# EugenHotaj/pytorch-generative

Measured on AMD Instinct MI355X. Metric: training images/sec (ImageGPT 8-block/4-head/16-embed, 28x28x1), higher is better.
Workload: dtype f32; 1 GPU; BASELINE.json configs[1]: ImageGPT 8 blocks / 4 heads / 16 embed on 28x28x1 binarised-MNIST-shaped synthetic; one step = zero_grad + fwd + BCE + bwd + global grad-norm + Adam + lr decay (reference trainer.py:173-193); per_gpu_batch=1024, global_batch=1024, parallelism=dp1, launch=hipGraph replay

## Files before the change

### include/pg_hip.h

```cpp
#ifndef PG_HIP_H_
#define PG_HIP_H_

#include <stddef.h>
#include <stdint.h>

#ifdef __cplusplus
extern "C" {
#endif

#define PG_ABI_VERSION 2

#define PG_EINVAL (-1)
#define PG_ESHAPE (-2)

#define PG_MAX_TAPS 64

#define PG_ACT_NONE 0
#define PG_ACT_RELU 1
#define PG_ACT_ELU 2
#define PG_ACT_GELU 3
#define PG_ACT_ELU_OUT 4

#define PG_GATE_TANH 0
#define PG_GATE_IDENTITY 1
// ... 170 lines not shown
                    void* stream);
size_t pg_mlp_gelu_bwd_workspace_floats(int N, int L);

int pg_gpt_block_head_fwd(const float* x, const float* ln_w, const float* ln_b, const float* wq,
                          const float* bq, const float* wkv, const float* bkv, float* qkv, int N,
                          int C, int L, float eps, void* stream);
int pg_gpt_block_head_bwd(const float* x, const float* ln_w, const float* ln_b, const float* wq,
                          const float* wkv, const float* dqkv, const float* gx, float* dx,
                          float* dln_w, float* dln_b, float* dwq, float* dbq, float* dwkv,
                          float* dbkv, int N, int C, int L, float eps, float* workspace,
                          size_t workspace_floats, void* stream);
size_t pg_gpt_block_head_bwd_workspace_floats(int N, int L);
int pg_gpt_block_tail_fwd(const float* o, const float* x, const float* wp, const float* bp,
                          const float* ln_w, const float* ln_b, const float* w1, const float* b1,
                          const float* w2, const float* b2, float* x_new, int N, int C, int Hd,
                          int L, float eps, void* stream);
int pg_gpt_block_tail_bwd(const float* o, const float* x, const float* wp, const float* bp,
                          const float* ln_w, const float* ln_b, const float* w1, const float* b1,
                          const float* w2, const float* dx_new, float* d_o, float* gx, float* dwp,
                          float* dbp, float* dln_w, float* dln_b, float* dw1, float* db1,
                          float* dw2, float* db2, int N, int C, int Hd, int L, float eps,
                          float* workspace, size_t workspace_floats, void* stream);
size_t pg_gpt_block_tail_bwd_workspace_floats(int N, int L);
int pg_gpt_block_tail_bwd_partial(const float* o, const float* x, const float* wp, const float* bp,
                                  const float* ln_w, const float* ln_b, const float* w1, const float* b1,
                                  const float* w2, const float* dx_new, float* d_o, float* gx, int N, int Cc,
                                  int Hd, int L, float eps, float* workspace, size_t workspace_floats,
                                  void* stream);
int pg_gpt_block_head_bwd_with_tail(const float* x, const float* ln_w, const float* ln_b, const float* wq,
                                    const float* wkv, const float* dqkv, const float* gx, float* dx,
                                    float* dln_w, float* dln_b, float* dwq, float* dbq, float* dwkv,
                                    float* dbkv, int N, int Cc, int L, float eps, float* workspace,
                                    size_t workspace_floats, const float* tail_workspace, float* t_dw1,
                                    float* t_db1, float* t_dw2, float* t_db2, float* t_dwp, float* t_dbp,
                                    float* t_dln_w, float* t_dln_b, void* stream);
int pg_gpt_block_head_bwd_partial(const float* x, const float* ln_w, const float* ln_b, const float* wq, const float* wkv,
                                  const float* dqkv, const float* gx, float* dx, int N, int C, int L, float eps,
                                  float* workspace, size_t workspace_floats, void* stream);
int pg_gpt_blocks_reduce(int n_blocks, const float* const* head_ws, const float* const* tail_ws, float* const* grads,
                         int N, int C, int L, void* stream);

int pg_sample_embed(const float* canvas, const float* pos, const float* w, const float* b, float* out,
                    int N, int Cin, int H, int W, int Cout, int KH, int KW, int r, int c, int ld,
                    const int* pos_dev, void* stream);
int pg_attn_decode(const float* qkv, float* k_cache, float* v_cache, float* o, int N, int heads,
                   int L, int p, int dk, int dv, int ld, int strict, const int* pos_dev,
// ... 76 lines not shown
```

### pytorch-generative_amd/csrc/gpt_block.hip

```cpp
#include <stdlib.h>

#include "common.h"
#include "gpt_ends.h"

namespace {

typedef float f32x4 __attribute__((ext_vector_type(4)));
#define MFMA16(A, B, C) __builtin_amdgcn_mfma_f32_16x16x4f32((A), (B), (C), 0, 0, 0)

constexpr int C = 16, HD = 64, QKV = 48;
constexpr int GB_THREADS = 256;
constexpr int TS = 20;
constexpr float INV_C = 1.f / 16.f;

constexpr int TB_WAVE_ROWS = 2 * HD + 4 * C;
constexpr int T_W1 = 0, T_B1 = T_W1 + HD * C, T_W2 = T_B1 + HD, T_B2 = T_W2 + C * HD, T_WP = T_B2 + C,
              T_BP = T_WP + C * C, T_G2 = T_BP + C, T_BE2 = T_G2 + C, T_PART = T_BE2 + C;
constexpr int H_WQ = 0, H_WKV = H_WQ + C * C, H_BQ = H_WKV + 2 * C * C, H_BKV = H_BQ + C,
              H_G1 = H_BKV + 2 * C, H_BE1 = H_G1 + C, H_PART = H_BE1 + C;

struct BlockArgs {
  const float* x; const float* g1; const float* be1; const float* wq; const float* bq;
  const float* wkv; const float* bkv; float* qkv; const float* dqkv; const float* gx; float* dx;
  const float* o; const float* wp; const float* bp; const float* g2; const float* be2;
// ... 59 lines not shown
};
__device__ __forceinline__ void prefetch_fence() { __builtin_amdgcn_sched_barrier(0); }
constexpr int waitcnt_gfx9(int vm, int exp, int lgkm) { return ((vm & 0x30) << 10) | (vm & 0xF) | ((exp & 7) << 4) | ((lgkm & 0xF) << 8); }
#if defined(__HIP_DEVICE_COMPILE__) && !defined(__GFX9__)
#error "wait_prologue_loads() encodes s_waitcnt for gfx9; re-derive the immediate for another target"
#endif
__device__ __forceinline__ void wait_prologue_loads() {
  constexpr int VMCNT0_ONLY = waitcnt_gfx9( 0,  7,  15);
  static_assert(VMCNT0_ONLY == 0x0F70, "gfx9 s_waitcnt vmcnt(0)");
  __builtin_amdgcn_s_waitcnt(VMCNT0_ONLY);
}
__device__ __forceinline__ void lds_put_tile(float* t, int j, int g, const f32x4& v) {
#pragma unroll
  for (int r = 0; r < 4; ++r) t[(4 * g + r) * TS + j] = v[r];
}
__device__ __forceinline__ f32x4 lds_row4(const float* t, int row, int g) {
  return *reinterpret_cast<const f32x4*>(t + row * TS + 4 * g);
}

__device__ __forceinline__ const float* qkv_row(const BlockArgs& a, int ch) {
  return ch < C ? a.wq + ch * C : a.wkv + (ch - C) * C;
}

__global__ void __launch_bounds__(GB_THREADS) head_fwd_kernel(const BlockArgs a) {
  const int lane = threadIdx.x & 63, j = lane & 15, g = lane >> 4;
  const int wave = blockIdx.x * (GB_THREADS / 64) + __builtin_amdgcn_readfirstlane(threadIdx.x >> 6);
  const int nwaves = gridDim.x * (GB_THREADS / 64);
  float wf[3][4];
  f32x4 bias[3];
#pragma unroll
  for (int m = 0; m < 3; ++m) {
#pragma unroll
    for (int r = 0; r < 4; ++r) {
      wf[m][r] = qkv_row(a, 16 * m + j)[4 * g + r];
      const int ch = 16 * m + 4 * g + r;
      bias[m][r] = ch < C ? a.bq[ch] : a.bkv[ch - C];
    }
  }
  const f32x4 gam = load_vec(a.g1, g), bet = load_vec(a.be1, g);
  if (wave >= a.total_tiles) return;
  TileWalk tw(a, wave, nwaves);
  f32x4 xv = load_tile(a.x + tw.base(C, a.L) + j, a.L, g);
  wait_prologue_loads();
  for (;;) {
    const TileWalk nx = tw.next();
    const bool more = nx.n < a.N;
    const f32x4 xn = load_tile(a.x + (more ? nx : tw).base(C, a.L) + j, a.L, g);
    prefetch_fence();
    const Ln s = ln_stats(xv, a.eps);
    f32x4 y;
#pragma unroll
    for (int r = 0; r < 4; ++r) y[r] = fmaf(s.xhat[r], gam[r], bet[r]);
    float* qb = a.qkv + tw.base(QKV, a.L) + j;
#pragma unroll
    for (int m = 0; m < 3; ++m) {
      f32x4 out = bias[m];
#pragma unroll
      for (int r = 0; r < 4; ++r) out = MFMA16(wf[m][r], y[r], out);
      store_tile(qb + (size_t)(16 * m) * a.L, a.L, g, out);
    }
    if (!more) break;
    xv = xn;
    tw = nx;
  }
}

__global__ void __launch_bounds__(GB_THREADS) head_bwd_kernel(const BlockArgs a) {
  extern __shared__ float4 lds4[];
  float* lds = reinterpret_cast<float*>(lds4);
  const int lane = threadIdx.x & 63, j = lane & 15, g = lane >> 4;
  const int wv = __builtin_amdgcn_readfirstlane(threadIdx.x >> 6);
  const int wave = blockIdx.x * (GB_THREADS / 64) + wv;
  const int nwaves = gridDim.x * (GB_THREADS / 64);
  float* ty = lds + (size_t)wv * (C + QKV) * TS;
  float* tq = ty + C * TS;

  float wt[3][4];
#pragma unroll
  for (int m = 0; m < 3; ++m) {
#pragma unroll
    for (int r = 0; r < 4; ++r) wt[m][r] = qkv_row(a, 16 * m + 4 * g + r)[j];
  }
  const f32x4 gam = load_vec(a.g1, g), bet = load_vec(a.be1, g);
// ... 67 lines not shown
  __syncthreads();
  float* mine = lds + (size_t)wv * H_PART;
#pragma unroll
  for (int m = 0; m < 3; ++m) {
#pragma unroll
    for (int r = 0; r < 4; ++r) {
      const int ch = 16 * m + 4 * g + r;
      mine[H_WQ + ch * C + j] = accw[m][r];
      const float b = jsum16(accb[m][r]);
      if (j == 0) mine[H_BQ + ch] = b;
    }
  }
#pragma unroll
  for (int r = 0; r < 4; ++r) {
    const float dg = jsum16(dgam[r]), db = jsum16(dbet[r]);
    if (j == 0) { mine[H_G1 + 4 * g + r] = dg; mine[H_BE1 + 4 * g + r] = db; }
  }
  __syncthreads();
  float* prow = a.part + (size_t)blockIdx.x * H_PART;
  for (int i = threadIdx.x; i < H_PART; i += GB_THREADS)
    prow[i] = (lds[i] + lds[H_PART + i]) + (lds[2 * H_PART + i] + lds[3 * H_PART + i]);
}

__global__ void __launch_bounds__(GB_THREADS) tail_fwd_kernel(const BlockArgs a) {
  const int lane = threadIdx.x & 63, j = lane & 15, g = lane >> 4;
  const int wave = blockIdx.x * (GB_THREADS / 64) + __builtin_amdgcn_readfirstlane(threadIdx.x >> 6);
  const int nwaves = gridDim.x * (GB_THREADS / 64);
  float wpf[4], w1f[4][4], w2f[4][4];
  f32x4 b1r[4];
#pragma unroll
  for (int r = 0; r < 4; ++r) wpf[r] = a.wp[j * C + 4 * g + r];
#pragma unroll
  for (int m = 0; m < 4; ++m) {
#pragma unroll
    for (int r = 0; r < 4; ++r) {
      w1f[m][r] = a.w1[(16 * m + j) * C + 4 * g + r];
      w2f[m][r] = a.w2[j * HD + 16 * m + 4 * g + r];
      b1r[m][r] = a.b1[16 * m + 4 * g + r];
    }
  }
  const f32x4 bpv = load_vec(a.bp, g), b2v = load_vec(a.b2, g);
  const f32x4 gam = load_vec(a.g2, g), bet = load_vec(a.be2, g);
  if (wave >= a.total_tiles) return;
  TileWalk tw(a, wave, nwaves);
  size_t off = tw.base(C, a.L) + j;
  f32x4 xv = load_tile(a.x + off, a.L, g);
  f32x4 ov = load_tile(a.o + off, a.L, g);
  wait_prologue_loads();
  for (;;) {
    const TileWalk nx = tw.next();
    const bool more = nx.n < a.N;
    const size_t offn = (more ? nx : tw).base(C, a.L) + j;
    const f32x4 xn = load_tile(a.x + offn, a.L, g);
    const f32x4 on = load_tile(a.o + offn, a.L, g);
    prefetch_fence();
    f32x4 xm = xv + bpv;
#pragma unroll
    for (int r = 0; r < 4; ++r) xm = MFMA16(wpf[r], ov[r], xm);
    const Ln s = ln_stats(xm, a.eps);
    f32x4 y;
#pragma unroll
    for (int r = 0; r < 4; ++r) y[r] = fmaf(s.xhat[r], gam[r], bet[r]);
    f32x4 h[4];
#pragma unroll
    for (int m = 0; m < 4; ++m) {
      h[m] = b1r[m];
#pragma unroll
      for (int r = 0; r < 4; ++r) h[m] = MFMA16(w1f[m][r], y[r], h[m]);
    }
    f32x4 out = (xm + b2v) + xv;
#pragma unroll
    for (int m = 0; m < 4; ++m) {
#pragma unroll
      for (int r = 0; r < 4; ++r) out = MFMA16(w2f[m][r], gelu_f(h[m][r]), out);
    }
    store_tile(a.xnew + off, a.L, g, out);
    if (!more) break;
    xv = xn;
    ov = on;
    off = offn;
    tw = nx;
  }
}

__global__ void __launch_bounds__(GB_THREADS) tail_bwd_kernel(const BlockArgs a) {
  extern __shared__ float4 lds4[];
  float* lds = reinterpret_cast<float*>(lds4);
  const int lane = threadIdx.x & 63, j = lane & 15, g = lane >> 4;
  const int wv = __builtin_amdgcn_readfirstlane(threadIdx.x >> 6);
  const int wave = blockIdx.x * (GB_THREADS / 64) + wv;
  const int nwaves = gridDim.x * (GB_THREADS / 64);
  float* tg = lds + (size_t)wv * TB_WAVE_ROWS * TS;
  float* th = tg + HD * TS;
  float* ty = th + HD * TS;
  float* tx = ty + C * TS;
  float* td = tx + C * TS;
  float* to = td + C * TS;

  float* wl = lds + (size_t)4 * TB_WAVE_ROWS * TS;
// ... 289 lines not shown
      const float* p = a.part + col[k];
      int r = rg;
      for (; r + 32 < a.rows; r += 64) {
        a0 += p[(size_t)r * a.stride];
        a1 += p[(size_t)(r + 32) * a.stride];
      }
      if (r < a.rows) a0 += p[(size_t)r * a.stride];
    }
  }
  red[rg][sl] = a0 + a1;
  __syncthreads();
  if (rg != 0 || s >= ncol) return;
  float acc = 0.f;
#pragma unroll
  for (int r = 0; r < 32; ++r) acc += red[r][sl];
  int begin = 0;
  for (int k = 0; k < a.nseg; ++k) {
    if (s < a.end[k]) { a.dst[k][s - begin] += acc; return; }
    begin = a.end[k];
  }
}

int grid_blocks(int which, int N, int L) {
  struct Cfg { int cap[4]; int mt[2]; };
  static const Cfg cfg = []() {
    Cfg c = {{2048, 1024, 2048, 512},
             {1, 2}};
    if (const char* e = PG_AB_ENV("PG_BLOCK_GRID")) {
      int v[4];
      if (sscanf(e, "%d,%d,%d,%d", &v[0], &v[1], &v[2], &v[3]) == 4 && v[0] > 0 && v[1] > 0 && v[2] > 0 && v[3] > 0)
        for (int i = 0; i < 4; ++i) c.cap[i] = v[i];
    }
    if (const char* e = PG_AB_ENV("PG_BLOCK_MINTILES")) {
      int f = 0, b = 0;
      if (sscanf(e, "%d,%d", &f, &b) == 2 && f > 0 && b > 0) { c.mt[0] = f; c.mt[1] = b; }
    }
    return c;
  }();
  const int* cap = cfg.cap;
  const int* mt_cfg = cfg.mt;
  const int min_tiles = (which & 1) ? mt_cfg[1] : mt_cfg[0];
  const long tiles = (long)N * (L / 16);
  long b = (tiles + 4 * min_tiles - 1) / (4 * min_tiles);
  if (b > cap[which]) b = cap[which];
  return b < 1 ? 1 : (int)b;
}
int bwd_blocks(int N, int L) { return grid_blocks(3, N, L); }

int check_shape(const char* who, int N, int Cc, int L) {
  PG_REQUIRE(N > 0 && L > 0, PG_EINVAL, "%s: non-positive dimension", who);
  PG_REQUIRE(Cc == C, PG_ESHAPE, "%s: only C = 16 is instantiated (got %d)", who, Cc);
  PG_REQUIRE(L % 16 == 0, PG_ESHAPE, "%s: L=%d is not a multiple of 16", who, L);
  return 0;
}
// ... 198 lines not shown
  }
  an.n = nj;
  an.first[nj] = nb;
  hipLaunchKernelGGL(seg_reduceM_kernel, dim3((unsigned)nb), dim3(256), 0, (hipStream_t)stream, an);
  PG_LAUNCH_CHECK("pg_gpt_model_reduce");
  return 0;
}

PG_EXPORT int pg_gpt_block_tail_fwd(const float* o, const float* x, const float* wp, const float* bp,
                                    const float* ln_w, const float* ln_b, const float* w1, const float* b1,
                                    const float* w2, const float* b2, float* x_new, int N, int Cc, int Hd,
                                    int L, float eps, void* stream) {
  PG_REQUIRE(o && x && wp && bp && ln_w && ln_b && w1 && b1 && w2 && b2 && x_new, PG_EINVAL,
             "pg_gpt_block_tail_fwd: null pointer");
  int rc = check_shape("pg_gpt_block_tail_fwd", N, Cc, L);
  if (rc) return rc;
  PG_REQUIRE(Hd == HD, PG_ESHAPE, "pg_gpt_block_tail_fwd: only hidden = 64 is instantiated (got %d)", Hd);
  BlockArgs a = {};
  a.o = o; a.x = x; a.wp = wp; a.bp = bp; a.g2 = ln_w; a.be2 = ln_b; a.w1 = w1; a.b1 = b1; a.w2 = w2;
  a.b2 = b2; a.xnew = x_new;
  set_geometry(a, N, L, eps);
  hipLaunchKernelGGL(tail_fwd_kernel, dim3((unsigned)grid_blocks(2, N, L)), dim3(GB_THREADS), 0, (hipStream_t)stream, a);
  PG_LAUNCH_CHECK("pg_gpt_block_tail_fwd");
  return 0;
}

namespace {
int tail_bwd_impl(const float* o, const float* x, const float* wp, const float* bp,
                                    const float* ln_w, const float* ln_b, const float* w1, const float* b1,
                                    const float* w2, const float* dx_new, float* d_o, float* gx,
                                    float* dwp, float* dbp, float* dln_w, float* dln_b, float* dw1,
                                    float* db1, float* dw2, float* db2, int N, int Cc, int Hd, int L,
                                    float eps, float* workspace, size_t workspace_floats, bool reduce_now, void* stream) {
  PG_REQUIRE(o && x && wp && bp && ln_w && ln_b && w1 && b1 && w2 && dx_new && d_o && gx && dwp && dbp &&
                 dln_w && dln_b && dw1 && db1 && dw2 && db2 && workspace, PG_EINVAL,
             "pg_gpt_block_tail_bwd: null pointer");
  int rc = check_shape("pg_gpt_block_tail_bwd", N, Cc, L);
  if (rc) return rc;
  PG_REQUIRE(Hd == HD, PG_ESHAPE, "pg_gpt_block_tail_bwd: only hidden = 64 is instantiated (got %d)", Hd);
  PG_REQUIRE(workspace_floats >= pg_gpt_block_tail_bwd_workspace_floats(N, L), PG_EINVAL,
             "pg_gpt_block_tail_bwd: workspace too small");
  PG_REQUIRE(al16(o) && al16(dx_new), PG_EINVAL, "pg_gpt_block_tail_bwd: o / dx_new must be 16-byte aligned");
  BlockArgs a = {};
  a.o = o; a.x = x; a.wp = wp; a.bp = bp; a.g2 = ln_w; a.be2 = ln_b; a.w1 = w1; a.b1 = b1; a.w2 = w2;
  a.dxnew = dx_new; a.d_o = d_o; a.gx_out = gx; a.part = workspace;
  set_geometry(a, N, L, eps);
// ... 37 lines not shown
```

### pytorch-generative_amd/pytorch_generative_amd/_lib.py

```python

import ctypes
import os

_HERE = os.path.dirname(os.path.abspath(__file__))
LIB_PATH = os.environ.get("PG_HIP_LIB") or os.path.join(_HERE, "lib", "libpg_hip.so")

ABI_VERSION = 2

c_f = ctypes.c_void_p
c_i = ctypes.c_int
c_l = ctypes.c_long
c_z = ctypes.c_size_t
c_s = ctypes.c_void_p
c_ip = ctypes.POINTER(ctypes.c_int)
c_flt = ctypes.c_float

SIGNATURES = {
    "pg_abi_version": (c_i, []),
    "pg_last_error": (ctypes.c_char_p, []),
    "pg_conv2d_taps": (
        c_i,
        [c_f, c_f, c_f, c_f, c_f, c_i, c_i, c_i, c_i, c_i, c_i, c_i, c_i, c_ip, c_ip, c_i, c_f, c_i,
         c_s],
    ),
# ... 26 lines not shown
    "pg_conv2d_wgrad_workspace_floats": (c_z, [c_i, c_i, c_i]),
    "pg_mul_inplace": (c_i, [c_f, c_f, c_z, c_s]),
    "pg_nchw_layernorm_fwd": (c_i, [c_f, c_f, c_f, c_f, c_f, c_f, c_i, c_i, c_i, c_flt, c_s]),
    "pg_nchw_layernorm_bwd": (
        c_i, [c_f, c_f, c_f, c_f, c_f, c_f, c_f, c_f, c_i, c_i, c_i, c_f, c_z, c_s]),
    "pg_gpt_block_head_fwd": (c_i, [c_f] * 8 + [c_i, c_i, c_i, c_flt, c_s]),
    "pg_gpt_block_head_bwd": (c_i, [c_f] * 14 + [c_i, c_i, c_i, c_flt, c_f, c_z, c_s]),
    "pg_gpt_block_head_bwd_workspace_floats": (c_z, [c_i, c_i]),
    "pg_gpt_block_head_bwd_partial": (c_i, [c_f] * 8 + [c_i, c_i, c_i, c_flt, c_f, c_z, c_s]),
    "pg_gpt_blocks_reduce": (c_i, [c_i, ctypes.POINTER(ctypes.c_void_p), ctypes.POINTER(ctypes.c_void_p),
                                   ctypes.POINTER(ctypes.c_void_p), c_i, c_i, c_i, c_s]),
    "pg_gpt_stem_fwd": (c_i, [c_f] * 5 + [c_i, c_i, c_i, c_i, c_s]),
    "pg_gpt_stem_bwd_plan": (c_i, [c_i, c_i, c_i, c_i, c_ip, c_ip]),
    "pg_gpt_stem_bwd_workspace_floats": (c_z, [c_i, c_i, c_i, c_i]),
    "pg_gpt_stem_bwd": (c_i, [c_f] * 4 + [c_i, c_i, c_i, c_i, c_f, c_z, c_s]),
    "pg_gpt_out_head_fwd": (c_i, [c_f] * 6 + [c_i, c_i, c_i, c_i, c_flt, c_i, c_s]),
    "pg_gpt_out_head_bwd_rows": (c_i, [c_i, c_i, c_i]),
    "pg_gpt_out_head_bwd": (c_i, [c_f] * 6 + [c_i, c_i, c_i, c_i, c_flt, c_i, c_f, c_z, c_s]),
    "pg_gpt_model_reduce": (c_i, [c_i, ctypes.POINTER(ctypes.c_void_p), ctypes.POINTER(ctypes.c_void_p),
                                  ctypes.POINTER(ctypes.c_void_p), c_i, c_i, c_i, c_f, c_i, c_i,
                                  ctypes.POINTER(ctypes.c_void_p), c_f, c_i, c_i, c_i, c_i,
                                  ctypes.POINTER(ctypes.c_void_p), c_s]),
    "pg_gpt_block_tail_fwd": (c_i, [c_f] * 11 + [c_i, c_i, c_i, c_i, c_flt, c_s]),
    "pg_gpt_block_tail_bwd": (c_i, [c_f] * 20 + [c_i, c_i, c_i, c_i, c_flt, c_f, c_z, c_s]),
    "pg_gpt_block_tail_bwd_workspace_floats": (c_z, [c_i, c_i]),
    "pg_gpt_block_tail_bwd_partial": (c_i, [c_f] * 12 + [c_i, c_i, c_i, c_i, c_flt, c_f, c_z, c_s]),
    "pg_gpt_block_head_bwd_with_tail": (c_i, [c_f] * 14 + [c_i, c_i, c_i, c_flt, c_f, c_z] + [c_f] * 9 + [c_s]),
    "pg_sample_embed": (c_i, [c_f] * 5 + [c_i] * 10 + [c_f, c_s]),
    "pg_attn_decode": (c_i, [c_f] * 4 + [c_i] * 8 + [c_f, c_s]),
    "pg_mlp_gelu_fwd": (c_i, [c_f, c_f, c_f, c_f, c_f, c_f, c_f, c_i, c_i, c_i, c_i, c_s]),
    "pg_mlp_gelu_bwd": (
        c_i, [c_f, c_f, c_f, c_f, c_f, c_f, c_f, c_f, c_f, c_f, c_i, c_i, c_i, c_i, c_f, c_z, c_s]),
    "pg_mlp_gelu_bwd_workspace_floats": (c_z, [c_i, c_i]),
    "pg_nchw_layernorm_bwd_res": (
        c_i, [c_f, c_f, c_f, c_f, c_f, c_f, c_f, c_f, c_f, c_i, c_i, c_i, c_f, c_z, c_s]),
    "pg_nchw_layernorm_bwd_workspace_floats": (c_z, [c_i, c_i, c_i]),
    "pg_causal_attn_fwd": (
        c_i,
        [c_f, c_f, c_f, c_f, c_f, c_i, c_i, c_i, c_i, c_i, c_l, c_l, c_l, c_l, c_i, c_s],
    ),
    "pg_causal_attn_bwd": (
        c_i,
        [c_f, c_f, c_f, c_f, c_f, c_f, c_f, c_f, c_f, c_f, c_i, c_i, c_i, c_i, c_i, c_l, c_l, c_l,
         c_l, c_l, c_l, c_l, c_l, c_i, c_s],
    ),
    "pg_causal_attn_bwd_dq": (
# ... 154 lines not shown
```

### pytorch-generative_amd/pytorch_generative_amd/models/autoregressive/image_gpt.py

```python

import os

import torch
from torch import nn

from pytorch_generative_amd import _lib
from pytorch_generative_amd import nn as pg_nn
from pytorch_generative_amd import ops
from pytorch_generative_amd.models import base

_BLOCK_CHAIN = os.environ.get("PG_BLOCK_CHAIN", "1") != "0"


class TransformerBlock(nn.Module):
    def __init__(self, n_channels, n_attention_heads):
        super().__init__()
        self._ln1 = pg_nn.NCHWLayerNorm(n_channels)
        self._ln2 = pg_nn.NCHWLayerNorm(n_channels)
        self._attn = pg_nn.CausalAttention(
            in_channels=n_channels,
            n_heads=n_attention_heads,
            embed_channels=n_channels,
            out_channels=n_channels,
        )
        self._out = nn.Sequential(
            pg_nn.Conv2d(in_channels=n_channels, out_channels=4 * n_channels, kernel_size=1),
            nn.GELU(),
            pg_nn.Conv2d(in_channels=4 * n_channels, out_channels=n_channels, kernel_size=1),
        )

    def _fused_ok(self, x):
        return ops.gpt_block_supported(x, self._ln1, self._attn._q, self._attn._kv, self._attn._proj,
                                       self._ln2, self._out[0], self._out[2])

    def forward_plus_input(self, x, chain=None, flush=False):
        if not self._fused_ok(x):
            return ops.add(x, self.forward(x))
        attn = self._attn
        pair = {}
        if chain is not None:
            pair["chain"], pair["flush"] = chain, flush
        qkv, xs = ops.gpt_block_head(x, self._ln1, attn._q, attn._kv, pair)
        o = ops.causal_attention_qkv(qkv, attn._n_heads, attn._embed_channels, attn._out_channels,
                                     attn._mask_center)
        return ops.gpt_block_tail(o, xs, attn._proj, self._ln2, self._out[0], self._out[2], pair)

    def forward(self, x):
        y, x = self._ln1(x, skip=True)
        x = self._attn(y, res=x)
        y, x = self._ln2(x, skip=True)
        if ops.mlp_gelu_supported(y, self._out[0], self._out[2]):
            return ops.mlp_gelu(y, self._out[0], self._out[2], res=x)
        hidden = self._out[0](y)
        return self._out[2](hidden, in_act="gelu", res=x)


class ImageGPT(base.AutoregressiveModel):
    def __init__(
        self,
        in_channels=1,
        out_channels=1,
        in_size=28,
        n_transformer_blocks=8,
        n_attention_heads=4,
        n_embedding_channels=16,
        sample_fn=None,
    ):
        super().__init__(sample_fn)
# ... 93 lines not shown
                current = canvas[:, :, row, col]
                canvas[:, :, row, col] = torch.where(current < 0, drawn, current)
        if return_logits:
            return canvas, torch.stack(all_logits)
        return canvas

    def forward(self, x):
        img, blocks, grad = x, list(self._transformer), torch.is_grad_enabled()
        fuse_stem = ops.gpt_stem_supported(img, self._pos, self._input)
        stem_flushes = fuse_stem and grad and any(p.requires_grad for p in (self._pos, self._input.weight, self._input.bias))
        if fuse_stem:
            x0_grad = stem_flushes
            probe = torch.empty(1, self._input.weight.shape[0], img.shape[2], img.shape[3], device="meta")
        else:
            x = probe = self._input(ops.add_broadcast_batch(img, self._pos))
            x0_grad = x.requires_grad
        chain = None
        if (ops.DEFER_BLOCK_REDUCE and _BLOCK_CHAIN and grad and x0_grad and len(blocks) > 1
                and all(b._fused_ok(probe) for b in blocks)
                and (stem_flushes or all(ops._sink(p) is not None for b in blocks for p in b.parameters()))):
            chain = ops.new_block_chain()
        if fuse_stem:
            x = self._input(img, pos=self._pos, chain=chain if stem_flushes else None)
        for i, block in enumerate(blocks):
            x = block.forward_plus_input(x, chain, flush=(i == 0 and not stem_flushes))
        if ops.gpt_out_head_supported(x, self._ln, self._out):
            return self._out(x, pre_ln=self._ln, chain=chain if stem_flushes else None)
        return self._out(self._ln(x))


def reproduce(n_epochs=457, batch_size=64, log_dir="/tmp/run", n_gpus=1, device_id=0,
              debug_loader=None):
    from pytorch_generative_amd import recipes

    return recipes.run(
        lambda: ImageGPT(in_channels=1, out_channels=1, in_size=28, n_transformer_blocks=8,
                         n_attention_heads=2, n_embedding_channels=64),
        loaders=recipes.binarized_mnist, loss_fn=recipes.bce_loss, lr=5e-3, lr_decay=0.999977,
        n_epochs=n_epochs, batch_size=batch_size, log_dir=log_dir, n_gpus=n_gpus,
        device_id=device_id, debug_loader=debug_loader)
```

### pytorch-generative_amd/pytorch_generative_amd/ops/gpt_block.py

```python

import os

import torch

from pytorch_generative_amd import _lib
from pytorch_generative_amd.ops._common import _chk, _p, _sink, _stream, zeros, zeros_like


FUSE_MLP = os.environ.get("PG_FUSE_MLP", "1") != "0"


def mlp_gelu_supported(x, conv1, conv2):
    if not FUSE_MLP or conv1.bias is None or conv2.bias is None:
        return False
    w1, w2 = conv1.weight, conv2.weight
    return (tuple(w1.shape) == (64, 16, 1, 1) and tuple(w2.shape) == (16, 64, 1, 1)
            and x.shape[1] == 16 and (x.shape[2] * x.shape[3]) % 16 == 0)


class _MlpGelu(torch.autograd.Function):
    @staticmethod
    def forward(ctx, x, w1, b1, w2, b2, res, sinks):
        lib = _lib.load()
        x = _chk(x, "mlp_gelu.x")
# ... 28 lines not shown
            else:
                t = zeros((c,), x.device) if like is None else zeros_like(like)
                grads.append(t)
                outs.append(t)
        ws_n = lib.pg_mlp_gelu_bwd_workspace_floats(n, h * w)
        ws = torch.empty(ws_n, device=x.device, dtype=torch.float32)
        _lib.check(
            lib.pg_mlp_gelu_bwd(x.data_ptr(), w1.data_ptr(), b1.data_ptr(), w2.data_ptr(),
                                dy.data_ptr(), dx.data_ptr(), grads[0].data_ptr(),
                                grads[1].data_ptr(), grads[2].data_ptr(), grads[3].data_ptr(), n, c,
                                hd, h * w, ws.data_ptr(), ws_n, _stream()),
            "pg_mlp_gelu_bwd",
        )
        return dx, outs[0], outs[1], outs[2], outs[3], (dy if ctx.has_res else None), None


def mlp_gelu(x, conv1, conv2, res=None):
    sinks = (_sink(conv1.weight), _sink(conv1.bias), _sink(conv2.weight), _sink(conv2.bias))
    return _MlpGelu.apply(x, conv1.weight, conv1.bias, conv2.weight, conv2.bias, res, sinks)


FUSE_BLOCK = os.environ.get("PG_FUSE_BLOCK", "1") != "0"
DEFER_BLOCK_REDUCE = os.environ.get("PG_BLOCK_REDUCE_MERGED", "1") != "0"


def _grad_targets(params):
    tgt, ret = [], []
    for p in params:
        sink = _sink(p)
        if sink is not None:
            tgt.append(sink)
            ret.append(None)
        else:
            z = zeros_like(p)
            tgt.append(z)
            ret.append(z)
    return tgt, ret


_open_chains = []


def new_block_chain():
    import weakref

    class _Chain(dict):
# ... 8 lines not shown
def assert_no_pending_block_reductions():
    for r in _open_chains:
        c = r()
        if c is not None and (c["jobs"] or c.get("out") is not None):
            raise RuntimeError(f"{len(c['jobs']) + (c.get('out') is not None)} deferred ImageGPT weight-gradient reductions were "
                               "never flushed: the backward that flushes them (the stem's, else the first block's) did not run "
                               "(set PG_BLOCK_REDUCE_MERGED=0 to reduce per block)")


def flush_block_reductions(chain, n, c, L):
    import ctypes

    lib = _lib.load()
    jobs = chain["jobs"]
    for i in range(0, len(jobs), 8):
        grp = jobs[i:i + 8]
        hw = (ctypes.c_void_p * len(grp))(*[j[0].data_ptr() for j in grp])
        tw = (ctypes.c_void_p * len(grp))(*[j[1].data_ptr() for j in grp])
        gr = (ctypes.c_void_p * (14 * len(grp)))(*[ptr for j in grp for ptr in j[2]])
        _lib.check(lib.pg_gpt_blocks_reduce(len(grp), hw, tw, gr, n, c, L, _stream()), "pg_gpt_blocks_reduce")
    jobs.clear()


class _GPTBlockHead(torch.autograd.Function):

    @staticmethod
    def forward(ctx, x, lnw, lnb, wq, bq, wkv, bkv, eps, params, pair=None):
        lib = _lib.load()
        ctx.pair = pair
        x_in = x
        x = _chk(x, "gpt_block_head.x")
        n, c, h, w = x.shape
        qkv = torch.empty((n, 3 * c, h, w), device=x.device, dtype=torch.float32)
        _lib.check(
            lib.pg_gpt_block_head_fwd(x.data_ptr(), lnw.data_ptr(), lnb.data_ptr(), wq.data_ptr(),
                                      bq.data_ptr(), wkv.data_ptr(), bkv.data_ptr(), qkv.data_ptr(),
                                      n, c, h * w, eps, _stream()),
            "pg_gpt_block_head_fwd",
        )
        ctx.save_for_backward(x, lnw, lnb, wq, wkv)
        ctx.eps, ctx.params = eps, params
        return qkv, x_in

    @staticmethod
    def backward(ctx, dqkv, gx):
        lib = _lib.load()
        x, lnw, lnb, wq, wkv = ctx.saved_tensors
        n, c, h, w = x.shape
        pending = ctx.pair.pop("tail", None) if ctx.pair is not None else None
        chain = ctx.pair.get("chain") if ctx.pair is not None else None
        flusher = chain is not None and bool(ctx.pair.get("flush"))
        if dqkv is None:
            if flusher and chain["jobs"]:
                flush_block_reductions(chain, n, c, h * w)
            if pending is not None:
                raise RuntimeError("gpt_block_head: a deferred tail reduction is pending but the head has no gradient")
            return gx, None, None, None, None, None, None, None, None, None
        dqkv = _chk(dqkv, "gpt_block_head.dqkv")
        gx = zeros_like(x) if gx is None else _chk(gx, "gpt_block_head.gx")
        dx = torch.empty_like(x)
        tgt, ret = _grad_targets(ctx.params)
        ws_n = lib.pg_gpt_block_head_bwd_workspace_floats(n, h * w)
# ... 14 lines not shown
                flush_block_reductions(chain, n, c, h * w)
            return (dx, *ret, None, None, None)
        if flusher and chain["jobs"]:
            flush_block_reductions(chain, n, c, h * w)
        if pending is not None:
            t_ws, t = pending
            _lib.check(
                lib.pg_gpt_block_head_bwd_with_tail(*head_args, t_ws.data_ptr(), t[4].data_ptr(), t[5].data_ptr(),
                                                    t[6].data_ptr(), t[7].data_ptr(), t[0].data_ptr(),
                                                    t[1].data_ptr(), t[2].data_ptr(), t[3].data_ptr(), _stream()),
                "pg_gpt_block_head_bwd_with_tail",
            )
        else:
            _lib.check(lib.pg_gpt_block_head_bwd(*head_args, _stream()), "pg_gpt_block_head_bwd")
        return (dx, *ret, None, None, None)


class _GPTBlockTail(torch.autograd.Function):

    @staticmethod
    def forward(ctx, o, x, wp, bp, lnw, lnb, w1, b1, w2, b2, eps, params, pair=None):
        lib = _lib.load()
        ctx.pair = pair
        o = _chk(o, "gpt_block_tail.o")
        x = _chk(x, "gpt_block_tail.x")
        n, c, h, w = x.shape
        x_new = torch.empty_like(x)
        _lib.check(
            lib.pg_gpt_block_tail_fwd(o.data_ptr(), x.data_ptr(), wp.data_ptr(), bp.data_ptr(),
                                      lnw.data_ptr(), lnb.data_ptr(), w1.data_ptr(), b1.data_ptr(),
                                      w2.data_ptr(), b2.data_ptr(), x_new.data_ptr(), n, c,
                                      w1.shape[0], h * w, eps, _stream()),
            "pg_gpt_block_tail_fwd",
        )
        ctx.save_for_backward(o, x, wp, bp, lnw, lnb, w1, b1, w2)
        ctx.eps, ctx.params = eps, params
        return x_new

    @staticmethod
    def backward(ctx, d):
        lib = _lib.load()
        o, x, wp, bp, lnw, lnb, w1, b1, w2 = ctx.saved_tensors
        d = _chk(d, "gpt_block_tail.dx_new")
        n, c, h, w = x.shape
        d_o, gx = torch.empty_like(o), torch.empty_like(x)
        tgt, ret = _grad_targets(ctx.params)
        ws_n = lib.pg_gpt_block_tail_bwd_workspace_floats(n, h * w)
        ws = torch.empty(ws_n, device=x.device, dtype=torch.float32)
        if ctx.pair is not None and DEFER_BLOCK_REDUCE and all(r is None for r in ret):
            _lib.check(
                lib.pg_gpt_block_tail_bwd_partial(o.data_ptr(), x.data_ptr(), wp.data_ptr(), bp.data_ptr(),
                                                  lnw.data_ptr(), lnb.data_ptr(), w1.data_ptr(), b1.data_ptr(),
                                                  w2.data_ptr(), d.data_ptr(), d_o.data_ptr(), gx.data_ptr(), n, c,
                                                  w1.shape[0], h * w, ctx.eps, ws.data_ptr(), ws_n, _stream()),
                "pg_gpt_block_tail_bwd_partial",
            )
            ctx.pair["tail"] = (ws, tgt)
# ... 8 lines not shown
                                      ctx.eps, ws.data_ptr(), ws_n, _stream()),
            "pg_gpt_block_tail_bwd",
        )
        return (d_o, gx, *ret, None, None, None)


def gpt_block_supported(x, ln1, q, kv, proj, ln2, fc1, fc2):
    if not FUSE_BLOCK or x.shape[1] != 16 or (x.shape[2] * x.shape[3]) % 16 != 0:
        return False
    shapes = (tuple(q.weight.shape), tuple(kv.weight.shape), tuple(proj.weight.shape),
              tuple(fc1.weight.shape), tuple(fc2.weight.shape))
    if shapes != ((16, 16, 1, 1), (32, 16, 1, 1), (16, 16, 1, 1), (64, 16, 1, 1), (16, 64, 1, 1)):
        return False
    if any(m.bias is None for m in (q, kv, proj, fc1, fc2)):
        return False
    return tuple(ln1.normalized_shape) == (16,) and tuple(ln2.normalized_shape) == (16,)


def gpt_block_head(x, ln1, q, kv, pair=None):
    params = (ln1.weight, ln1.bias, q.weight, q.bias, kv.weight, kv.bias)
    return _GPTBlockHead.apply(x, *params, float(ln1.eps), params, pair)


def gpt_block_tail(o, x, proj, ln2, fc1, fc2, pair=None):
    params = (proj.weight, proj.bias, ln2.weight, ln2.bias, fc1.weight, fc1.bias, fc2.weight, fc2.bias)
    return _GPTBlockTail.apply(o, x, *params, float(ln2.eps), params, pair)


class _NCHWLayerNorm(torch.autograd.Function):
    @staticmethod
    def forward(ctx, x, gamma, beta, eps, gg, gb, with_skip=False):
        lib = _lib.load()
        x_in = x
        x = _chk(x, "layernorm.x")
        n, c, h, w = x.shape
        if gamma.numel() != c:
            raise ValueError(f"NCHWLayerNorm: normalized_shape {gamma.numel()} != channels {c}")
        y = torch.empty_like(x)
        mean = torch.empty(n * h * w, device=x.device, dtype=torch.float32)
        rstd = torch.empty_like(mean)
        _lib.check(
            lib.pg_nchw_layernorm_fwd(x.data_ptr(), gamma.data_ptr(), beta.data_ptr(), y.data_ptr(),
                                      mean.data_ptr(), rstd.data_ptr(), n, c, h * w, eps, _stream()),
            "pg_nchw_layernorm_fwd",
        )
        ctx.save_for_backward(x, gamma, mean, rstd)
        ctx.gg, ctx.gb = gg, gb
        if with_skip:
            return y, x_in
# ... 47 lines not shown
```

Baseline: 106,200 images/s.

## Fuse block tail forward with next block's head QKV projection

Adds a tail_head_fwd kernel that computes a block's MLP tail and then immediately applies the next block's LayerNorm and QKV projection on the same register tile. This removes one kernel launch per block boundary and the re-read of x_new from global memory. Python plumbing passes the precomputed qkv through a boundary dict and checks it against the next head's inputs and parameters. The fused kernel holds more weight fragments in registers (launch bounds hint of 3), which may reduce occupancy.

```diff
diff --git a/include/pg_hip.h b/include/pg_hip.h
--- a/include/pg_hip.h
+++ b/include/pg_hip.h
@@ -216,6 +216,12 @@
                           float* dw2, float* db2, int N, int C, int Hd, int L, float eps,
                           float* workspace, size_t workspace_floats, void* stream);
 size_t pg_gpt_block_tail_bwd_workspace_floats(int N, int L);
+int pg_gpt_block_tail_head_fwd(const float* o, const float* x, const float* wp, const float* bp,
+                               const float* ln_w, const float* ln_b, const float* w1, const float* b1,
+                               const float* w2, const float* b2, float* x_new, const float* next_ln_w,
+                               const float* next_ln_b, const float* next_wq, const float* next_bq,
+                               const float* next_wkv, const float* next_bkv, float* next_qkv, int N, int C,
+                               int Hd, int L, float eps, void* stream);
 int pg_gpt_block_tail_bwd_partial(const float* o, const float* x, const float* wp, const float* bp,
                                   const float* ln_w, const float* ln_b, const float* w1, const float* b1,
                                   const float* w2, const float* dx_new, float* d_o, float* gx, int N, int Cc,
diff --git a/pytorch-generative_amd/csrc/gpt_block.hip b/pytorch-generative_amd/csrc/gpt_block.hip
--- a/pytorch-generative_amd/csrc/gpt_block.hip
+++ b/pytorch-generative_amd/csrc/gpt_block.hip
@@ -105,22 +105,44 @@
   return ch < C ? a.wq + ch * C : a.wkv + (ch - C) * C;
 }
 
+struct HeadFrags {
+  float wf[3][4]; f32x4 bias[3], gam, bet;
+  __device__ __forceinline__ HeadFrags(const BlockArgs& a, int j, int g) {
+#pragma unroll
+    for (int m = 0; m < 3; ++m) {
+#pragma unroll
+      for (int r = 0; r < 4; ++r) {
+        wf[m][r] = qkv_row(a, 16 * m + j)[4 * g + r];
+        const int ch = 16 * m + 4 * g + r;
+        bias[m][r] = ch < C ? a.bq[ch] : a.bkv[ch - C];
+      }
+    }
+    gam = load_vec(a.g1, g);
+    bet = load_vec(a.be1, g);
+  }
+};
+__device__ __forceinline__ void head_chain(const f32x4& xv, const HeadFrags& f, float eps, f32x4 (&out)[3]) {
+  const Ln s = ln_stats(xv, eps);
+  f32x4 y;
+#pragma unroll
+  for (int r = 0; r < 4; ++r) y[r] = fmaf(s.xhat[r], f.gam[r], f.bet[r]);
+#pragma unroll
+  for (int m = 0; m < 3; ++m) {
+    out[m] = f.bias[m];
+#pragma unroll
+    for (int r = 0; r < 4; ++r) out[m] = MFMA16(f.wf[m][r], y[r], out[m]);
+  }
+}
+__device__ __forceinline__ void store_qkv_tiles(float* __restrict__ qb, int L, int g, const f32x4 (&q)[3]) {
+#pragma unroll
+  for (int m = 0; m < 3; ++m) store_tile(qb + (size_t)(16 * m) * L, L, g, q[m]);
+}
+
 __global__ void __launch_bounds__(GB_THREADS) head_fwd_kernel(const BlockArgs a) {
   const int lane = threadIdx.x & 63, j = lane & 15, g = lane >> 4;
   const int wave = blockIdx.x * (GB_THREADS / 64) + __builtin_amdgcn_readfirstlane(threadIdx.x >> 6);
   const int nwaves = gridDim.x * (GB_THREADS / 64);
-  float wf[3][4];
-  f32x4 bias[3];
-#pragma unroll
-  for (int m = 0; m < 3; ++m) {
-#pragma unroll
-    for (int r = 0; r < 4; ++r) {
-      wf[m][r] = qkv_row(a, 16 * m + j)[4 * g + r];
-      const int ch = 16 * m + 4 * g + r;
-      bias[m][r] = ch < C ? a.bq[ch] : a.bkv[ch - C];
-    }
-  }
-  const f32x4 gam = load_vec(a.g1, g), bet = load_vec(a.be1, g);
+  const HeadFrags hf(a, j, g);
   if (wave >= a.total_tiles) return;
   TileWalk tw(a, wave, nwaves);
   f32x4 xv = load_tile(a.x + tw.base(C, a.L) + j, a.L, g);
@@ -130,18 +152,9 @@
     const bool more = nx.n < a.N;
     const f32x4 xn = load_tile(a.x + (more ? nx : tw).base(C, a.L) + j, a.L, g);
     prefetch_fence();
-    const Ln s = ln_stats(xv, a.eps);
-    f32x4 y;
-#pragma unroll
-    for (int r = 0; r < 4; ++r) y[r] = fmaf(s.xhat[r], gam[r], bet[r]);
-    float* qb = a.qkv + tw.base(QKV, a.L) + j;
-#pragma unroll
-    for (int m = 0; m < 3; ++m) {
-      f32x4 out = bias[m];
-#pragma unroll
-      for (int r = 0; r < 4; ++r) out = MFMA16(wf[m][r], y[r], out);
-      store_tile(qb + (size_t)(16 * m) * a.L, a.L, g, out);
-    }
+    f32x4 q[3];
+    head_chain(xv, hf, a.eps, q);
+    store_qkv_tiles(a.qkv + tw.base(QKV, a.L) + j, a.L, g, q);
     if (!more) break;
     xv = xn;
     tw = nx;
@@ -255,25 +268,58 @@
     prow[i] = (lds[i] + lds[H_PART + i]) + (lds[2 * H_PART + i] + lds[3 * H_PART + i]);
 }
 
+struct TailFrags {
+  float wpf[4];
+  float w1f[4][4];
+  float w2f[4][4];
+  f32x4 b1r[4], bpv, b2v, gam, bet;
+  __device__ __forceinline__ TailFrags(const BlockArgs& a, int j, int g) {
+#pragma unroll
+    for (int r = 0; r < 4; ++r) wpf[r] = a.wp[j * C + 4 * g + r];
+#pragma unroll
+    for (int m = 0; m < 4; ++m) {
+#pragma unroll
+      for (int r = 0; r < 4; ++r) {
+        w1f[m][r] = a.w1[(16 * m + j) * C + 4 * g + r];
+        w2f[m][r] = a.w2[j * HD + 16 * m + 4 * g + r];
+        b1r[m][r] = a.b1[16 * m + 4 * g + r];
+      }
+    }
+    bpv = load_vec(a.bp, g);
+    b2v = load_vec(a.b2, g);
+    gam = load_vec(a.g2, g);
+    bet = load_vec(a.be2, g);
+  }
+};
+__device__ __forceinline__ f32x4 tail_chain(const f32x4& xv, const f32x4& ov, const TailFrags& f, float eps) {
+  f32x4 xm = xv + f.bpv;
+#pragma unroll
+  for (int r = 0; r < 4; ++r) xm = MFMA16(f.wpf[r], ov[r], xm);
+  const Ln s = ln_stats(xm, eps);
+  f32x4 y;
+#pragma unroll
+  for (int r = 0; r < 4; ++r) y[r] = fmaf(s.xhat[r], f.gam[r], f.bet[r]);
+  f32x4 h[4];
+#pragma unroll
+  for (int m = 0; m < 4; ++m) {
+    h[m] = f.b1r[m];
+#pragma unroll
+    for (int r = 0; r < 4; ++r) h[m] = MFMA16(f.w1f[m][r], y[r], h[m]);
+  }
+  f32x4 out = (xm + f.b2v) + xv;
+#pragma unroll
+  for (int m = 0; m < 4; ++m) {
+#pragma unroll
+    for (int r = 0; r < 4; ++r) out = MFMA16(f.w2f[m][r], gelu_f(h[m][r]), out);
+  }
+  return out;
+}
+
 __global__ void __launch_bounds__(GB_THREADS) tail_fwd_kernel(const BlockArgs a) {
   const int lane = threadIdx.x & 63, j = lane & 15, g = lane >> 4;
   const int wave = blockIdx.x * (GB_THREADS / 64) + __builtin_amdgcn_readfirstlane(threadIdx.x >> 6);
   const int nwaves = gridDim.x * (GB_THREADS / 64);
-  float wpf[4], w1f[4][4], w2f[4][4];
-  f32x4 b1r[4];
-#pragma unroll
-  for (int r = 0; r < 4; ++r) wpf[r] = a.wp[j * C + 4 * g + r];
-#pragma unroll
-  for (int m = 0; m < 4; ++m) {
-#pragma unroll
-    for (int r = 0; r < 4; ++r) {
-      w1f[m][r] = a.w1[(16 * m + j) * C + 4 * g + r];
-      w2f[m][r] = a.w2[j * HD + 16 * m + 4 * g + r];
-      b1r[m][r] = a.b1[16 * m + 4 * g + r];
-    }
-  }
-  const f32x4 bpv = load_vec(a.bp, g), b2v = load_vec(a.b2, g);
-  const f32x4 gam = load_vec(a.g2, g), bet = load_vec(a.be2, g);
+  const TailFrags tf(a, j, g);
   if (wave >= a.total_tiles) return;
   TileWalk tw(a, wave, nwaves);
   size_t off = tw.base(C, a.L) + j;
@@ -287,27 +333,39 @@
     const f32x4 xn = load_tile(a.x + offn, a.L, g);
     const f32x4 on = load_tile(a.o + offn, a.L, g);
     prefetch_fence();
-    f32x4 xm = xv + bpv;
-#pragma unroll
-    for (int r = 0; r < 4; ++r) xm = MFMA16(wpf[r], ov[r], xm);
-    const Ln s = ln_stats(xm, a.eps);
-    f32x4 y;
-#pragma unroll
-    for (int r = 0; r < 4; ++r) y[r] = fmaf(s.xhat[r], gam[r], bet[r]);
-    f32x4 h[4];
-#pragma unroll
-    for (int m = 0; m < 4; ++m) {
-      h[m] = b1r[m];
-#pragma unroll
-      for (int r = 0; r < 4; ++r) h[m] = MFMA16(w1f[m][r], y[r], h[m]);
-    }
-    f32x4 out = (xm + b2v) + xv;
-#pragma unroll
-    for (int m = 0; m < 4; ++m) {
-#pragma unroll
-      for (int r = 0; r < 4; ++r) out = MFMA16(w2f[m][r], gelu_f(h[m][r]), out);
-    }
+    store_tile(a.xnew + off, a.L, g, tail_chain(xv, ov, tf, a.eps));
+    if (!more) break;
+    xv = xn;
+    ov = on;
+    off = offn;
+    tw = nx;
+  }
+}
+
+__global__ void __launch_bounds__(GB_THREADS, 3) tail_head_fwd_kernel(const BlockArgs a) {
+  const int lane = threadIdx.x & 63, j = lane & 15, g = lane >> 4;
+  const int wave = blockIdx.x * (GB_THREADS / 64) + __builtin_amdgcn_readfirstlane(threadIdx.x >> 6);
+  const int nwaves = gridDim.x * (GB_THREADS / 64);
+  const TailFrags tf(a, j, g);
+  const HeadFrags hf(a, j, g);
+  if (wave >= a.total_tiles) return;
+  TileWalk tw(a, wave, nwaves);
+  size_t off = tw.base(C, a.L) + j;
+  f32x4 xv = load_tile(a.x + off, a.L, g);
+  f32x4 ov = load_tile(a.o + off, a.L, g);
+  wait_prologue_loads();
+  for (;;) {
+    const TileWalk nx = tw.next();
+    const bool more = nx.n < a.N;
+    const size_t offn = (more ? nx : tw).base(C, a.L) + j;
+    const f32x4 xn = load_tile(a.x + offn, a.L, g);
+    const f32x4 on = load_tile(a.o + offn, a.L, g);
+    prefetch_fence();
+    const f32x4 out = tail_chain(xv, ov, tf, a.eps);
     store_tile(a.xnew + off, a.L, g, out);
+    f32x4 q[3];
+    head_chain(out, hf, a.eps, q);
+    store_qkv_tiles(a.qkv + tw.base(QKV, a.L) + j, a.L, g, q);
     if (!more) break;
     xv = xn;
     ov = on;
@@ -643,14 +701,16 @@
 }
 
 int grid_blocks(int which, int N, int L) {
-  struct Cfg { int cap[4]; int mt[2]; };
+  struct Cfg { int cap[5]; int mt[2]; };
   static const Cfg cfg = []() {
-    Cfg c = {{2048, 1024, 2048, 512},
+    Cfg c = {{2048, 1024, 2048, 512,
+              1536},
              {1, 2}};
     if (const char* e = PG_AB_ENV("PG_BLOCK_GRID")) {
-      int v[4];
-      if (sscanf(e, "%d,%d,%d,%d", &v[0], &v[1], &v[2], &v[3]) == 4 && v[0] > 0 && v[1] > 0 && v[2] > 0 && v[3] > 0)
-        for (int i = 0; i < 4; ++i) c.cap[i] = v[i];
+      int v[5];
+      const int got = sscanf(e, "%d,%d,%d,%d,%d", &v[0], &v[1], &v[2], &v[3], &v[4]);
+      if (got >= 4 && v[0] > 0 && v[1] > 0 && v[2] > 0 && v[3] > 0 && (got == 4 || v[4] > 0))
+        for (int i = 0; i < got; ++i) c.cap[i] = v[i];
     }
     if (const char* e = PG_AB_ENV("PG_BLOCK_MINTILES")) {
       int f = 0, b = 0;
@@ -895,6 +955,27 @@
   set_geometry(a, N, L, eps);
   hipLaunchKernelGGL(tail_fwd_kernel, dim3((unsigned)grid_blocks(2, N, L)), dim3(GB_THREADS), 0, (hipStream_t)stream, a);
   PG_LAUNCH_CHECK("pg_gpt_block_tail_fwd");
+  return 0;
+}
+
+PG_EXPORT int pg_gpt_block_tail_head_fwd(const float* o, const float* x, const float* wp, const float* bp,
+                                         const float* ln_w, const float* ln_b, const float* w1, const float* b1,
+                                         const float* w2, const float* b2, float* x_new, const float* next_ln_w,
+                                         const float* next_ln_b, const float* next_wq, const float* next_bq,
+                                         const float* next_wkv, const float* next_bkv, float* next_qkv, int N, int Cc,
+                                         int Hd, int L, float eps, void* stream) {
+  PG_REQUIRE(o && x && wp && bp && ln_w && ln_b && w1 && b1 && w2 && b2 && x_new && next_ln_w && next_ln_b && next_wq &&
+                 next_bq && next_wkv && next_bkv && next_qkv, PG_EINVAL, "pg_gpt_block_tail_head_fwd: null pointer");
+  int rc = check_shape("pg_gpt_block_tail_head_fwd", N, Cc, L);
+  if (rc) return rc;
+  PG_REQUIRE(Hd == HD, PG_ESHAPE, "pg_gpt_block_tail_head_fwd: only hidden = 64 is instantiated (got %d)", Hd);
+  BlockArgs a = {};
+  a.o = o; a.x = x; a.wp = wp; a.bp = bp; a.g2 = ln_w; a.be2 = ln_b; a.w1 = w1; a.b1 = b1; a.w2 = w2;
+  a.b2 = b2; a.xnew = x_new;
+  a.g1 = next_ln_w; a.be1 = next_ln_b; a.wq = next_wq; a.bq = next_bq; a.wkv = next_wkv; a.bkv = next_bkv; a.qkv = next_qkv;
+  set_geometry(a, N, L, eps);
+  hipLaunchKernelGGL(tail_head_fwd_kernel, dim3((unsigned)grid_blocks(4, N, L)), dim3(GB_THREADS), 0, (hipStream_t)stream, a);
+  PG_LAUNCH_CHECK("pg_gpt_block_tail_head_fwd");
   return 0;
 }
 
diff --git a/pytorch-generative_amd/pytorch_generative_amd/_lib.py b/pytorch-generative_amd/pytorch_generative_amd/_lib.py
--- a/pytorch-generative_amd/pytorch_generative_amd/_lib.py
+++ b/pytorch-generative_amd/pytorch_generative_amd/_lib.py
@@ -72,6 +72,7 @@
                                   ctypes.POINTER(ctypes.c_void_p), c_f, c_i, c_i, c_i, c_i,
                                   ctypes.POINTER(ctypes.c_void_p), c_s]),
     "pg_gpt_block_tail_fwd": (c_i, [c_f] * 11 + [c_i, c_i, c_i, c_i, c_flt, c_s]),
+    "pg_gpt_block_tail_head_fwd": (c_i, [c_f] * 18 + [c_i, c_i, c_i, c_i, c_flt, c_s]),
     "pg_gpt_block_tail_bwd": (c_i, [c_f] * 20 + [c_i, c_i, c_i, c_i, c_flt, c_f, c_z, c_s]),
     "pg_gpt_block_tail_bwd_workspace_floats": (c_z, [c_i, c_i]),
     "pg_gpt_block_tail_bwd_partial": (c_i, [c_f] * 12 + [c_i, c_i, c_i, c_i, c_flt, c_f, c_z, c_s]),
diff --git a/pytorch-generative_amd/pytorch_generative_amd/models/autoregressive/image_gpt.py b/pytorch-generative_amd/pytorch_generative_amd/models/autoregressive/image_gpt.py
--- a/pytorch-generative_amd/pytorch_generative_amd/models/autoregressive/image_gpt.py
+++ b/pytorch-generative_amd/pytorch_generative_amd/models/autoregressive/image_gpt.py
@@ -33,17 +33,20 @@
         return ops.gpt_block_supported(x, self._ln1, self._attn._q, self._attn._kv, self._attn._proj,
                                        self._ln2, self._out[0], self._out[2])
 
-    def forward_plus_input(self, x, chain=None, flush=False):
+    def forward_plus_input(self, x, chain=None, flush=False, boundary=None, next_block=None):
         if not self._fused_ok(x):
             return ops.add(x, self.forward(x))
         attn = self._attn
         pair = {}
         if chain is not None:
             pair["chain"], pair["flush"] = chain, flush
+        if boundary is not None:
+            pair["boundary"] = boundary
+        nxt = None if next_block is None else (next_block._ln1, next_block._attn._q, next_block._attn._kv)
         qkv, xs = ops.gpt_block_head(x, self._ln1, attn._q, attn._kv, pair)
         o = ops.causal_attention_qkv(qkv, attn._n_heads, attn._embed_channels, attn._out_channels,
                                      attn._mask_center)
-        return ops.gpt_block_tail(o, xs, attn._proj, self._ln2, self._out[0], self._out[2], pair)
+        return ops.gpt_block_tail(o, xs, attn._proj, self._ln2, self._out[0], self._out[2], pair, nxt)
 
     def forward(self, x):
         y, x = self._ln1(x, skip=True)
@@ -183,8 +186,11 @@
             chain = ops.new_block_chain()
         if fuse_stem:
             x = self._input(img, pos=self._pos, chain=chain if stem_flushes else None)
+        fused = [b._fused_ok(probe) for b in blocks] if ops.gpt_block.FUSE_BOUNDARY else [False] * len(blocks)
+        boundary = {} if any(fused) else None
         for i, block in enumerate(blocks):
-            x = block.forward_plus_input(x, chain, flush=(i == 0 and not stem_flushes))
+            nxt = blocks[i + 1] if i + 1 < len(blocks) and fused[i] and fused[i + 1] else None
+            x = block.forward_plus_input(x, chain, flush=(i == 0 and not stem_flushes), boundary=boundary, next_block=nxt)
         if ops.gpt_out_head_supported(x, self._ln, self._out):
             return self._out(x, pre_ln=self._ln, chain=chain if stem_flushes else None)
         return self._out(self._ln(x))
diff --git a/pytorch-generative_amd/pytorch_generative_amd/ops/gpt_block.py b/pytorch-generative_amd/pytorch_generative_amd/ops/gpt_block.py
--- a/pytorch-generative_amd/pytorch_generative_amd/ops/gpt_block.py
+++ b/pytorch-generative_amd/pytorch_generative_amd/ops/gpt_block.py
@@ -74,6 +74,7 @@
 
 FUSE_BLOCK = os.environ.get("PG_FUSE_BLOCK", "1") != "0"
 DEFER_BLOCK_REDUCE = os.environ.get("PG_BLOCK_REDUCE_MERGED", "1") != "0"
+FUSE_BOUNDARY = os.environ.get("PG_FUSE_BOUNDARY", "1") != "0"
 
 
 def _grad_targets(params):
@@ -128,6 +129,17 @@
     jobs.clear()
 
 
+def _take_boundary_qkv(pair, x, head, eps):
+    boundary = pair.get("boundary") if pair is not None else None
+    entry = boundary.pop("qkv", None) if boundary is not None else None
+    if entry is None:
+        return None
+    x_new, version, params, e, qkv = entry
+    same = (x.data_ptr() == x_new.data_ptr() and x.shape == x_new.shape and x.stride() == x_new.stride()
+            and x._version == version and e == eps and len(params) == len(head) and all(a is b for a, b in zip(params, head)))
+    return qkv if same else None
+
+
 class _GPTBlockHead(torch.autograd.Function):
 
     @staticmethod
@@ -137,13 +149,15 @@
         x_in = x
         x = _chk(x, "gpt_block_head.x")
         n, c, h, w = x.shape
-        qkv = torch.empty((n, 3 * c, h, w), device=x.device, dtype=torch.float32)
-        _lib.check(
-            lib.pg_gpt_block_head_fwd(x.data_ptr(), lnw.data_ptr(), lnb.data_ptr(), wq.data_ptr(),
-                                      bq.data_ptr(), wkv.data_ptr(), bkv.data_ptr(), qkv.data_ptr(),
-                                      n, c, h * w, eps, _stream()),
-            "pg_gpt_block_head_fwd",
-        )
+        qkv = _take_boundary_qkv(pair, x, (lnw, lnb, wq, bq, wkv, bkv), eps)
+        if qkv is None:
+            qkv = torch.empty((n, 3 * c, h, w), device=x.device, dtype=torch.float32)
+            _lib.check(
+                lib.pg_gpt_block_head_fwd(x.data_ptr(), lnw.data_ptr(), lnb.data_ptr(), wq.data_ptr(),
+                                          bq.data_ptr(), wkv.data_ptr(), bkv.data_ptr(), qkv.data_ptr(),
+                                          n, c, h * w, eps, _stream()),
+                "pg_gpt_block_head_fwd",
+            )
         ctx.save_for_backward(x, lnw, lnb, wq, wkv)
         ctx.eps, ctx.params = eps, params
         return qkv, x_in
@@ -204,17 +218,30 @@
     def forward(ctx, o, x, wp, bp, lnw, lnb, w1, b1, w2, b2, eps, params, pair=None):
         lib = _lib.load()
         ctx.pair = pair
+        next_head = pair.pop("next_head", None) if pair is not None else None
         o = _chk(o, "gpt_block_tail.o")
         x = _chk(x, "gpt_block_tail.x")
         n, c, h, w = x.shape
         x_new = torch.empty_like(x)
-        _lib.check(
-            lib.pg_gpt_block_tail_fwd(o.data_ptr(), x.data_ptr(), wp.data_ptr(), bp.data_ptr(),
-                                      lnw.data_ptr(), lnb.data_ptr(), w1.data_ptr(), b1.data_ptr(),
-                                      w2.data_ptr(), b2.data_ptr(), x_new.data_ptr(), n, c,
-                                      w1.shape[0], h * w, eps, _stream()),
-            "pg_gpt_block_tail_fwd",
-        )
+        if next_head is not None:
+            qkv = torch.empty((n, 3 * c, h, w), device=x.device, dtype=torch.float32)
+            _lib.check(
+                lib.pg_gpt_block_tail_head_fwd(o.data_ptr(), x.data_ptr(), wp.data_ptr(), bp.data_ptr(),
+                                               lnw.data_ptr(), lnb.data_ptr(), w1.data_ptr(), b1.data_ptr(),
+                                               w2.data_ptr(), b2.data_ptr(), x_new.data_ptr(),
+                                               *(t.data_ptr() for t in next_head), qkv.data_ptr(), n, c,
+                                               w1.shape[0], h * w, eps, _stream()),
+                "pg_gpt_block_tail_head_fwd",
+            )
+            pair["boundary"]["qkv"] = (x_new, x_new._version, tuple(next_head), eps, qkv)
+        else:
+            _lib.check(
+                lib.pg_gpt_block_tail_fwd(o.data_ptr(), x.data_ptr(), wp.data_ptr(), bp.data_ptr(),
+                                          lnw.data_ptr(), lnb.data_ptr(), w1.data_ptr(), b1.data_ptr(),
+                                          w2.data_ptr(), b2.data_ptr(), x_new.data_ptr(), n, c,
+                                          w1.shape[0], h * w, eps, _stream()),
+                "pg_gpt_block_tail_fwd",
+            )
         ctx.save_for_backward(o, x, wp, bp, lnw, lnb, w1, b1, w2)
         ctx.eps, ctx.params = eps, params
         return x_new
@@ -269,9 +296,14 @@
     return _GPTBlockHead.apply(x, *params, float(ln1.eps), params, pair)
 
 
-def gpt_block_tail(o, x, proj, ln2, fc1, fc2, pair=None):
+def gpt_block_tail(o, x, proj, ln2, fc1, fc2, pair=None, next_head=None):
     params = (proj.weight, proj.bias, ln2.weight, ln2.bias, fc1.weight, fc1.bias, fc2.weight, fc2.bias)
-    return _GPTBlockTail.apply(o, x, *params, float(ln2.eps), params, pair)
+    eps = float(ln2.eps)
+    if next_head is not None and pair is not None and pair.get("boundary") is not None:
+        ln1, q, kv = next_head
+        if float(ln1.eps) == eps:
+            pair["next_head"] = (ln1.weight, ln1.bias, q.weight, q.bias, kv.weight, kv.bias)
+    return _GPTBlockTail.apply(o, x, *params, eps, params, pair)
 
 
 class _NCHWLayerNorm(torch.autograd.Function):
```

New measurement: 108,400 images/s (median of 6 runs). +2.1%, better.
